# sunwookim028/bwa-mem-gpu

Measured on AMD Instinct MI355X. Metric: reads/s aligned (150 bp PE vs hg38-scale 3100 Mbp synthetic genome), file to file (bwahip_stream_run), higher is better.
Workload: dtype u64

## Files before the change

### bwa-mem-gpu_amd/bwahip.py

```python
import ctypes as C
import os
import subprocess
import numpy as np

_HERE = os.path.dirname(os.path.abspath(__file__))
LIB_PATH = os.environ.get("BWAHIP_LIB") or os.path.join(_HERE, "libbwahip.so")
TOOLS = os.path.join(_HERE, "tools")


class Opt(C.Structure):
    _fields_ = [("max_mem_intv", C.c_uint64), ("a", C.c_int), ("b", C.c_int), ("o_del", C.c_int), ("e_del", C.c_int),
                ("o_ins", C.c_int), ("e_ins", C.c_int), ("pen_unpaired", C.c_int), ("pen_clip5", C.c_int),
                ("pen_clip3", C.c_int), ("w", C.c_int), ("zdrop", C.c_int), ("T", C.c_int), ("flag", C.c_int),
                ("min_seed_len", C.c_int), ("min_chain_weight", C.c_int), ("max_chain_extend", C.c_int),
                ("split_factor", C.c_float), ("split_width", C.c_int), ("max_occ", C.c_int), ("max_chain_gap", C.c_int),
                ("n_threads", C.c_int), ("chunk_size", C.c_int), ("mask_level", C.c_float), ("drop_ratio", C.c_float),
                ("XA_drop_ratio", C.c_float), ("mask_level_redun", C.c_float), ("mapQ_coef_len", C.c_float),
                ("mapQ_coef_fac", C.c_int), ("max_ins", C.c_int), ("max_matesw", C.c_int), ("max_XA_hits", C.c_int),
                ("max_XA_hits_alt", C.c_int), ("mat", C.c_int8 * 25)]


class Seq(C.Structure):
    _fields_ = [("l_seq", C.c_int), ("id", C.c_int), ("name", C.c_char_p), ("comment", C.c_char_p),
                ("seq", C.POINTER(C.c_char)), ("qual", C.c_char_p), ("sam", C.POINTER(C.c_char)),
# ... 1169 lines not shown
        return dup[:len(desc)]

    def kat_radix_sort(self, keys, key_bits=64):
        keys = np.ascontiguousarray(keys, dtype=np.uint64)
        idx = np.empty(len(keys), dtype=np.uint32)
        tile = C.c_int()
        _check(lib().bwahip_kat_radix_sort(self._h, len(keys), keys.ctypes.data, key_bits, idx.ctypes.data, C.byref(tile)), "bwahip_kat_radix_sort")
        return idx, tile.value

    def batch_run(self, opt=None):
        opt = opt or default_opt()
        nk = lib().bwahip_n_kernels()
        ms = (C.c_float * nk)()
        _check(lib().bwahip_batch_run(self._h, C.byref(opt), ms, nk), "bwahip_batch_run")
        return {lib().bwahip_kernel_name(i).decode(): float(ms[i]) for i in range(nk)}

    @staticmethod
    def stage_names():
        return ["k_smem(passes 1-2)+k_smem_heavy+k_smem3(pass 3)+k_intv_sort", "k_seeds", "k_chain(+k_chain_big,k_chain_flt)", "k_seed_sw (only with -W / reads > 700 bp)",
                "k_extend_spec+k_extend(+k_extend_big, dedup/patch)", "pe_rescue = PE: k_pestat + k_pe_prepare + k_pe_copy (insert sizes, lists; the rescue kernels k_matesw_sw / k_matesw start on the second stream)",
                "k_mark (mark primary) + PE: k_pair (pairing) beside the rescue kernels, then both for the rescued pairs",
                "k_cigar (mem_reg2aln: mapQ, CIGAR by ksw_global2 backtrack, NM/MD)", "k_sam size + scan + write (SAM text)"]

    @staticmethod
    def output_description(paired):
        return "SAM text of the batch in HBM (== seqs[i].sam of mem_process_seqs, " + ("paired-end: mate rescue, pairing, paired records)" if paired else "single-end)")

    def counters(self):
        buf = (C.c_uint64 * 32)()
        _check(lib().bwahip_batch_counters(self._h, buf, 32), "bwahip_batch_counters")
        names = ["extend", "blocks", "sa", "lf", "intv", "seeds", "cells", "max_extends", "chain_build_max", "chain_sort_max", "chain_flt_max",
                 "chain_write_max", "max_seeds", "max_chains", "ext_max", "ext_dedup_max", "heavy_blocks", "heavy_intv", "heavy_reads",
                 "dp_rows_1col", "dp_rows_ncol", "dedup_sort1_max", "dedup_loop_max", "dedup_sort2_max",
                 "pass3_blocks", "pass3_intv", "pass3_jumped", "ext_calls", "ext_diag", "smem_lookups", "smem_fallbacks", "_31"]
        return {k: int(buf[i]) for i, k in enumerate(names)}

    def kat_introsort(self, k64, score, qb, mode):
        k64 = np.ascontiguousarray(k64, dtype=np.int64); score = np.ascontiguousarray(score, dtype=np.int32); qb = np.ascontiguousarray(qb, dtype=np.int32)
        n = len(k64)
        a = np.empty(n, dtype=np.int32); b = np.empty(n, dtype=np.int32); st = np.zeros(2, dtype=np.int32)
        _check(lib().bwahip_kat_introsort(self._h, n, mode, k64.ctypes.data, score.ctypes.data, qb.ctypes.data, a.ctypes.data, b.ctypes.data, st.ctypes.data), "bwahip_kat_introsort")
        assert st[1] == 0
        return a, b, bool(st[0])

    def kat_mate_insert(self, list_off, list_words, step_off, step_hit, step_words, opt=None, mode=0, where=0):
        opt = opt or default_opt()
        list_off = np.ascontiguousarray(list_off, dtype=np.int64); step_off = np.ascontiguousarray(step_off, dtype=np.int64)
        list_words = np.ascontiguousarray(list_words, dtype=np.int64).reshape(-1, 19); step_words = np.ascontiguousarray(step_words, dtype=np.int64).reshape(-1, 19)
        step_hit = np.ascontiguousarray(step_hit, dtype=np.int32)
        n = len(list_off) - 1
        assert len(step_off) == n + 1 and len(list_words) >= list_off.max() and len(step_words) >= step_off.max() and len(step_hit) == len(step_words)
        out = np.zeros((max(0, int(list_off[-1] + step_off[-1])), 19), dtype=np.int64); out_n = np.zeros(n, dtype=np.int32); cnt = np.zeros((n, 3), dtype=np.int32)
        _check(lib().bwahip_kat_mate_insert(self._h, C.byref(opt), n, list_off.ctypes.data, list_words.ctypes.data, step_off.ctypes.data, step_hit.ctypes.data, step_words.ctypes.data,
                                            mode, where, out.ctypes.data, out_n.ctypes.data, cnt.ctypes.data), "bwahip_kat_mate_insert")
        return out, out_n, cnt

    def kat_occ4(self, k):
        k = np.ascontiguousarray(k, dtype=np.uint64)
        out = np.zeros((len(k), 4), dtype=np.uint64)
        _check(lib().bwahip_kat_occ4(self._h, len(k), k.ctypes.data, out.ctypes.data), "bwahip_kat_occ4")
        return out

    def kat_sa(self, k):
        k = np.ascontiguousarray(k, dtype=np.uint64)
        out = np.zeros(len(k), dtype=np.uint64)
        _check(lib().bwahip_kat_sa(self._h, len(k), k.ctypes.data, out.ctypes.data), "bwahip_kat_sa")
        return out
# ... 284 lines not shown
```

### bwa-mem-gpu_amd/csrc/bwahip_internal.h

```cpp
#pragma once
#include <hip/hip_runtime.h>
#include <stdint.h>
#include <stdio.h>
#include <stdlib.h>
#include <string.h>
#include <vector>
#include <string>
#include "../../include/bwahip.h"

#define HIP_TRY(expr) do { hipError_t e_ = (expr); if (e_ != hipSuccess) { \
	fprintf(stderr, "[bwahip] %s failed at %s:%d: %s\n", #expr, __FILE__, __LINE__, hipGetErrorString(e_)); \
	return BWAHIP_ENODEV; } } while (0)

struct DevAnn { int64_t offset; int32_t len; int32_t is_alt; };

struct DevIndex {
	const uint4 *bwt;
	const uint64_t *sa;
	const uint8_t *pac;
	const DevAnn *anns;
	uint64_t primary, L2[5], seq_len, n_sa;
	int64_t l_pac;
	int sa_intv, sa_shift, n_seqs;
	const uint4 *kmer; int kmer_k;
};
__host__ __device__ inline uint64_t kmer_off(int L) { return (0x5555555555555555ull & ((1ull << 2 * L) - 1)) - 1; }

struct DevOpt {
	int a, b, o_del, e_del, o_ins, e_ins, pen_clip5, pen_clip3, w, zdrop;
	int min_seed_len, split_width, max_occ, max_chain_gap, max_mem_intv, split_len;
	int min_chain_weight, max_chain_extend;
	float mask_level, drop_ratio, mask_level_redun;
	int8_t mat[25];
	int T, flag, pen_unpaired, max_ins, max_matesw, max_XA_hits, max_XA_hits_alt, mapQ_coef_fac;
	float XA_drop_ratio, mapQ_coef_len;
};

enum { CNT_EXTEND = 0, CNT_BLOCKS, CNT_SA, CNT_LF, CNT_INTV, CNT_SEEDS, CNT_CELLS, CNT_MAX_EXT ,
       CNT_HEAVY_BLOCKS = 16, CNT_HEAVY_INTV, CNT_HEAVY_READS, CNT_ROWS1 , CNT_ROWSN ,
       CNT_P3_BLOCKS = 24, CNT_P3_INTV, CNT_P3_JUMPED ,
       CNT_EXT_CALLS , CNT_EXT_DIAG ,
       CNT_SMEM_LOOKUPS , CNT_SMEM_FALLBACKS , CNT_N = 32 };
constexpr int CNT_SLOTS = 256;
#define BWAHIP_MISC_BYTES ((size_t)CNT_SLOTS * CNT_N * 8 + 64)
#ifdef __HIPCC__
__device__ __forceinline__ unsigned long long *cnt_row(unsigned long long *base)
{
	return base + (size_t)((blockIdx.x * (blockDim.x >> 6) + (threadIdx.x >> 6)) & (CNT_SLOTS - 1)) * CNT_N;
}
#endif

struct __attribute__((aligned(32))) DevIntv { uint64_t x0, x1, x2, info; };

struct __attribute__((aligned(16))) DevSeed { int64_t rbeg; int32_t qbeg, len; int32_t score, rid; };

struct DevChain {
	int64_t pos;
	int32_t seed_off, n;
	int32_t rid, w, kept, first, is_alt;
	float frac_rep;
};

struct DevReg {
	int64_t rb, re;
	float frac_rep;
	int32_t qb, qe, rid, score, truesc, sub, csub, sub_n, w, seedcov, seedlen0, n_comp, is_alt;
	int32_t pad;
};

#include <thread>
#include <vector>
template <class F> static inline void par_for_chunks(int64_t n, int nt, F f)
{
	if (nt <= 1 || n < 4096) { f((int64_t)0, n); return; }
	std::vector<std::thread> th;
// ... 119 lines not shown
	int64_t pad2;
};
static_assert(sizeof(DevAln) == 80 && sizeof(DevReg) == 80, "record sizes");
enum { NEED_REC = 1 , NEED_XA = 2 , NEED_H = 4  };
struct DevPes { int low, high, failed, pad; double avg, std; };
struct PeRead;

struct FinLaunch {
	DevIndex ix; DevOpt opt;
	int n_reads; const uint8_t *seq; const int64_t *off;
	int64_t n_processed;
	const double *logtab;
	const DevReg *regs; const int64_t *reg_base; const int *reg_n;
	FinReg *fregs, *fregs2; int *freg_n, *n_pri; int *scr;
	const uint8_t *resc_flag; const int *resc_pairs; int subset;
	int read_lo;
	uint8_t *need; int *xa_owner;
	int *task_n, *rec_n;
	const int64_t *task_base;
	int2 *tasks;
	int *fast_list, *dp_list, *list_n;
	int *aln_of_reg;
	DevAln *alns;
	uint8_t *pool; unsigned long long *pool_head; unsigned long long pool_cap;
	int *redo_list, *redo_n; uint8_t *big_z;
	unsigned *zslab;
	const uint8_t *qual; const int64_t *qual_off;
	const uint8_t *names; const int64_t *name_off; const uint8_t *comments; const int64_t *comment_off;
	const uint8_t *ctg_names; const int *ctg_name_off; const uint8_t *ctg_anno; const int *ctg_anno_off;
	const uint8_t *rg_id; int rg_len;
	int *sam_len; const int64_t *sam_off; uint8_t *sam;
	const DevAln **rec_list, **xa_list;
	const PeRead *pe_read; DevPes pes[4];
	int *err;
};
int launch_mark_primary(const FinLaunch &a, bool plan, int n_listed, hipStream_t st);
int launch_kat_mapq(const FinLaunch &a, int64_t n_slots, int *out2, hipStream_t st);
int launch_task_fill(const FinLaunch &a, hipStream_t st);
int launch_cigar(const FinLaunch &a, int n_fast, int n_dp, int max_len, hipStream_t st, hipStream_t st2, hipEvent_t fork, hipEvent_t join);
int launch_cigar_big(const FinLaunch &a, int grid, hipStream_t st);
size_t cigar_big_slab_bytes();
size_t cigar_zslab_bytes(int max_len, int n_dp);
int launch_sam(const FinLaunch &a, bool write, hipStream_t st, int read_lo = 0, int read_hi = -1);

struct PeRead {
	int mode;
	int h_reg;
	int alt_reg;
	int mapq;
	int extra_flag;
	int pad[3];
};
struct SwRes { int state , score, te, qe, score2, te2, tb, qb; };
struct PairLaunch {
	DevIndex ix; DevOpt opt;
	int n_reads; const uint8_t *seq; const int64_t *off;
	int64_t n_processed;
	const double *logtab;
	const DevReg *regs; const int64_t *reg_base; const int *reg_n;
	unsigned *hist;
	DevPes pes[4];
	const double *pair_tab; int tab_off[4];
	int *nb;
	int *pe_cap; const int64_t *pe_base;
	DevReg *pe_regs; int *pe_n;
	DevReg *pe_tmp; void *pe_keys; int *pe_idx;
	int *resc_list; int *resc_n;
	const int64_t *sw_base; int *sw_cnt; SwRes *sw_res; int *sw_tasks; int2 *sw_info; int *sw_n;
	int *sw_n8; int sw_cap;
	uint8_t *slab; size_t slab_stride;
	int incr_insert;
	unsigned int *queue;
	unsigned long long *counters;
	unsigned long long *paths;
	int *pair_dbg;
// ... 59 lines not shown
```

### bwa-mem-gpu_amd/csrc/ctx_internal.h

```cpp
#pragma once
#include "bwahip_internal.h"
#include "own.h"
#include "upload_once.h"
#include <atomic>
#include <memory>
#include <string>
#include <utility>

inline std::atomic<long> g_bwahip_reallocs{0};
inline std::atomic<int64_t> g_bwahip_live[6];

struct DevMem {
	static constexpr size_t slack = 256;
	static constexpr const char *what = "hipMalloc";
	static void *alloc(size_t bytes)
	{
		void *p = nullptr;
		if (hipMalloc(&p, bytes ? bytes : 1) != hipSuccess) { (void)hipGetLastError(); return nullptr; }
		++g_bwahip_live[0]; g_bwahip_live[1] += (int64_t)bytes;
		return p;
	}
	static void free(void *p, size_t bytes) { (void)hipFree(p); --g_bwahip_live[0]; g_bwahip_live[1] -= (int64_t)bytes; }
	static void count_sync() { ++g_bwahip_reallocs; }
};
// ... 34 lines not shown
	Stream() = default;
	Stream(Stream &&o) noexcept : s(o.s) { o.s = nullptr; }
	Stream &operator=(Stream &&o) noexcept { if (this != &o) { reset(); s = o.s; o.s = nullptr; } return *this; }
	~Stream() { reset(); }
	int make(unsigned flags = hipStreamNonBlocking)
	{
		reset();
		if (hipStreamCreateWithFlags(&s, flags) != hipSuccess) { (void)hipGetLastError(); s = nullptr; return BWAHIP_ENODEV; }
		++g_bwahip_live[5];
		return 0;
	}
	void reset() { if (s) { (void)hipStreamDestroy(s); --g_bwahip_live[5]; s = nullptr; } }
	operator hipStream_t() const { return s; }
};

struct Knobs {
	int intv_cap = 96;
	int smem_lanes = 1;
	int sa_intv = 1;
	int kmer_k = 14;
	int smem_skip = -1;
	int heavy_mult = -1;
	int chain_mid_max = 1536, chain_big_max = 3200, chain_glb_grid = 2048;
	int chain_big_min = 512;
	int rank_sort_min = 2;
	int spec_min_chains = 16;
	int ext_lds_window = 1 << 30;
	int ext_early_stop = 1;
	int ext_diag = 1;
	int sorted_piece_blocks = 1024;
	int gpu_final = 1;
	int gpu_pair = 1;
	int incr_insert = 1;
	int verbose = 0;
	int e2e_log = 0;
	const char *dump_ext = nullptr;
	void from_env()
	{
		auto geti = [](const char *k, int &v) { if (const char *e = getenv(k)) v = atoi(e); };
		geti("BWAHIP_INTV_CAP", intv_cap); geti("BWAHIP_SMEM_LANES", smem_lanes); geti("BWAHIP_HEAVY_MULT", heavy_mult); geti("BWAHIP_SMEM_SKIP", smem_skip); geti("BWAHIP_SA_INTV", sa_intv); geti("BWAHIP_KMER_K", kmer_k);
		geti("BWAHIP_CHAIN_BIG_MIN", chain_big_min); geti("BWAHIP_CHAIN_MID_MAX", chain_mid_max); geti("BWAHIP_CHAIN_BIG_MAX", chain_big_max); geti("BWAHIP_CHAIN_GLB_GRID", chain_glb_grid); geti("BWAHIP_RANK_SORT_MIN", rank_sort_min); geti("BWAHIP_SPEC_MIN_CHAINS", spec_min_chains); geti("BWAHIP_EXT_LDS_WINDOW", ext_lds_window); geti("BWAHIP_EXT_EARLY_STOP", ext_early_stop); geti("BWAHIP_EXT_DIAG", ext_diag); geti("BWAHIP_GPU_FINAL", gpu_final); geti("BWAHIP_GPU_PAIR", gpu_pair);
		verbose = getenv("BWAHIP_VERBOSE") != nullptr;
		e2e_log = getenv("BWAHIP_E2E_LOG") != nullptr;
		dump_ext = getenv("BWAHIP_DUMP_EXT");
		if (intv_cap < 2) intv_cap = 2;
		ext_early_stop = ext_early_stop != 0; ext_diag = ext_diag != 0;
		geti("BWAHIP_INCR_INSERT", incr_insert); incr_insert = incr_insert != 0;
		geti("BWAHIP_SORTED_PIECE_BLOCKS", sorted_piece_blocks);
		if (sorted_piece_blocks < 1 || sorted_piece_blocks > 4096) sorted_piece_blocks = 1024;
	}
};

struct BatchText {
	std::vector<int64_t> off, qoff, noff, coff;
	int64_t qtot = 0;
	bool any_comment = false;
	size_t sz_codes = 0, sz_qual = 0, sz_names = 0, sz_comm = 0;
};

struct BamSort {
	DevBuf raw, rec_cnt, rec_base, keys[2], idx[2], off, len, len_sorted, hist, hist_base, bits;
	DevBuf tmpl;
	float ms[3] = { 0, 0, 0 };
	int n_passes = 0;
};

struct Bgzf {
	DevBuf slots, mlen, moff, md, cnt;
};

enum class OutForm { Sam, Bam, BamSorted, Bgzf, BamSortedDup };
inline bool is_bam(OutForm f) { return f != OutForm::Sam; }
inline bool is_sorted(OutForm f) { return f == OutForm::BamSorted || f == OutForm::BamSortedDup; }

struct BatchIn {
	DevBuf d_seq, d_off, d_qual, d_qual_off, d_names, d_name_off, d_comments, d_comment_off;
	HostBuf h_stage;
	Event ev;
	int n = 0, max_len = 0; int64_t total_bases = 0; bool any_comment = false;
	const uint8_t *comments() const { return any_comment ? d_comments.as<uint8_t>() : nullptr; }
// ... 205 lines not shown
```

### bwa-mem-gpu_amd/csrc/final_rt.hip

```cpp
#include "ctx_internal.h"
#include <atomic>
#include <thread>
#include <math.h>
#include <algorithm>
#include <chrono>

#include <dlfcn.h>
typedef int (*host_final_fn)(bwahip_ctx*, const bwahip_opt_t*, int64_t, int, bwahip_seq_t*, const bwahip_pestat_t*);
static host_final_fn load_host_final()
{
	static host_final_fn fn = nullptr;
	static bool tried = false;
	if (tried) return fn;
	tried = true;
	Dl_info di;
	std::string path = "libbwahip_hostfinal.so";
	if (dladdr((const void*)&bwahip_version, &di) && di.dli_fname) {
		const std::string self = di.dli_fname;
		const size_t sl = self.rfind('/');
		if (sl != std::string::npos) path = self.substr(0, sl + 1) + path;
	}
	void *h = dlopen(path.c_str(), RTLD_NOW | RTLD_LOCAL);
	if (h) fn = (host_final_fn)dlsym(h, "bwahip_process_seqs_host");
	if (!fn) fprintf(stderr, "[bwahip] gpu_final / gpu_pair = 0 need the test library %s (%s)\n", path.c_str(), h ? "symbol missing" : dlerror());
// ... 132 lines not shown
	HIP_TRY(hipMemcpyAsync(&n_sw_tasks, pl.sw_n, 4, hipMemcpyDeviceToHost, c->stream));
	HIP_TRY(hipStreamSynchronize(c->stream));
	n_resc_out = n_resc;
	c->last_pe_counters[3] = (unsigned long long)n_resc;
	c->last_sw_tasks = (unsigned long long)n_sw_tasks + (unsigned long long)n_sw_tasks8;
	c->last_sw_ahead[0] = (unsigned long long)n_sw_tasks; c->last_sw_ahead[1] = (unsigned long long)n_sw_tasks8;
	if (n_resc > 0 || n_sw_tasks > 0 || n_sw_tasks8 > 0) {
		HIP_TRY(hipEventRecord(c->ev_fork, c->stream));
		HIP_TRY(hipStreamWaitEvent(c->stream2, c->ev_fork, 0));
		if ((rc = launch_matesw_sw(pl, n_sw_tasks, n_sw_tasks8, c->in->max_len, c->stream2))) return rc;
		if (n_resc > 0) {
			if ((rc = c->d_resc_ord.ensure(((size_t)3 * n_resc + 8) * 4)) || (rc = launch_resc_order(pl, n_resc, c->d_resc_ord.as<int>(), c->stream2))) return rc;
			const int grid = std::min(n_resc, 2048);
			pl.slab_stride = (matesw_slab_bytes(widest + c->in->max_len) + 255) & ~(size_t)255;
			if ((rc = c->d_ms_slab.ensure(pl.slab_stride * (size_t)grid))) return rc;
			pl.slab = c->d_ms_slab.as<uint8_t>();
			HIP_TRY(hipMemsetAsync(pl.queue, 0, 16, c->stream2));
			if ((rc = launch_matesw(pl, grid, c->stream2))) return rc;
		}
		HIP_TRY(hipEventRecord(c->ev_join, c->stream2));
	}
	return 0;
}

static int mark_prepare(bwahip_ctx *c, const bwahip_opt_t *opt, int n, int64_t n_processed, bool pe_lists, FinLaunch &f)
{
	int rc;
	const size_t R = (size_t)(c->total_regs ? c->total_regs : 1);
	if ((rc = c->d_fregs.ensure(R * sizeof(FinReg))) || (rc = c->d_fregs2.ensure(R * sizeof(FinReg))) || (rc = c->d_fscr.ensure(R * 16)) || (rc = c->d_need.ensure(R)) ||
	    (rc = c->d_xa_owner.ensure(R * 4)) || (rc = c->d_freg_n.ensure((size_t)n * 4)) || (rc = c->d_npri.ensure((size_t)n * 4)) || (rc = c->d_task_n.ensure((size_t)n * 4)) ||
	    (rc = c->d_rec_n.ensure((size_t)n * 4))) return rc;
	memset(&f, 0, sizeof f);
	f.ix = c->ix; f.opt = make_dev_opt(opt); f.n_reads = n;
	f.n_processed = n_processed; f.logtab = c->d_logtab.as<double>();
	f.regs = c->d_regs.as<DevReg>(); f.reg_base = c->d_reg_base.as<int64_t>(); f.reg_n = c->d_reg_n.as<int>();
	if (pe_lists) { f.regs = c->d_pe_regs.as<DevReg>(); f.reg_base = c->d_pe_base.as<int64_t>(); f.reg_n = c->d_pe_n.as<int>(); }
	f.fregs = c->d_fregs.as<FinReg>(); f.fregs2 = c->d_fregs2.as<FinReg>(); f.freg_n = c->d_freg_n.as<int>(); f.n_pri = c->d_npri.as<int>(); f.scr = c->d_fscr.as<int>();
	f.need = c->d_need.as<uint8_t>(); f.xa_owner = c->d_xa_owner.as<int>(); f.task_n = c->d_task_n.as<int>(); f.rec_n = c->d_rec_n.as<int>();
	return 0;
}

static int pair_wire(bwahip_ctx *c, const FinLaunch &f, int n, bool dbg, PairLaunch &pl)
{
	int rc;
	if ((rc = c->d_pe_read.ensure((size_t)n * sizeof(PeRead)))) return rc;
	pl.fregs = f.fregs; pl.fregs_w = f.fregs; pl.fregs_tmp = f.fregs2; pl.freg_n = f.freg_n; pl.n_pri = f.n_pri; pl.need = f.need; pl.xa_owner = f.xa_owner;
	pl.task_n = f.task_n; pl.rec_n = f.rec_n; pl.scr = f.scr; pl.pe_read = c->d_pe_read.as<PeRead>();
	if (dbg) {
		if ((rc = c->d_pair_dbg.ensure((size_t)(n / 2) * 12))) return rc;
		HIP_TRY(hipMemsetAsync(c->d_pair_dbg.p, 0, (size_t)(n / 2) * 12, c->stream));
		pl.pair_dbg = c->d_pair_dbg.as<int>();
	}
	return 0;
}

int run_final(bwahip_ctx *c, const bwahip_opt_t *opt, int64_t n_processed, const bwahip_pestat_t *pes0, bool timed, OutForm form, bool host_sam_off, bool pe_stage_stop)
{
	auto launch_out = [&](const FinLaunch &fl, bool write, int lo, int hi) {
		const bool pe_ = (opt->flag & BWAHIP_F_PE) != 0;
		return is_bam(form) ? (pe_ ? launch_bam_pe(fl, write, c->stream, lo, hi) : launch_bam(fl, write, c->stream, lo, hi)) : (pe_ ? launch_sam_pe(fl, write, c->stream, lo, hi) : launch_sam(fl, write, c->stream, lo, hi));
	};
	const int n = c->in->n;
	const bool pe = (opt->flag & BWAHIP_F_PE) != 0;
	BatchOut &o = *c->out;
	o.total = 0; o.n_rec = 0; o.n_blocks = 0; o.n_stored = 0; o.n_tmpl = 0; o.form = form; c->total_tasks = 0;
	const bool sorted = is_sorted(form);
	const bool bgzf = form == OutForm::Bgzf;
	if (n == 0) return 0;
	if (pe && (n & 1)) return BWAHIP_EINVAL;
	int rc;
	HIP_TRY(hipMemsetAsync(c->d_fmisc.p, 0, 256, c->stream));
	if (timed) HIP_TRY(hipEventRecord(c->ev[20], c->stream));
	PairLaunch pl;
	const DevOpt dopt_pe = make_dev_opt(opt);
	int n_resc = 0;
	if (pe && (rc = run_pe_rescue(c, opt, dopt_pe, n_processed, pes0, pl, n_resc))) return rc;
	FinLaunch f;
	if ((rc = mark_prepare(c, opt, n, n_processed, pe, f))) return rc;
	const size_t R = (size_t)(c->total_regs ? c->total_regs : 1);
	if ((rc = c->d_aln_of_reg.ensure(R * 4)) || (rc = c->d_rec_list.ensure(R * 8)) || (rc = c->d_xa_list.ensure(R * 8)) ||
	    (rc = c->d_task_base.ensure((size_t)(n + 1) * 8)) || (rc = c->d_sam_len.ensure((size_t)n * 4)) || (rc = o.d_sam_off.ensure((size_t)(n + 1) * 8))) return rc;
	{
		std::string rg = c->rg_id;
		rg.resize(rg.size() + 64, 0);
		if ((rc = dev_upload(c->d_rg, rg.data(), rg.size(), c->stream))) return rc;
	}
	f.seq = c->in->d_seq.as<uint8_t>(); f.off = c->in->d_off.as<int64_t>();
	f.task_base = c->d_task_base.as<int64_t>(); f.aln_of_reg = c->d_aln_of_reg.as<int>();
	f.rec_list = c->d_rec_list.as<const DevAln*>(); f.xa_list = c->d_xa_list.as<const DevAln*>();
	unsigned long long *pool_head = c->d_fmisc.as<unsigned long long>();
	f.pool_head = pool_head; f.redo_n = (int*)(pool_head + 1); f.err = (int*)(pool_head + 2);
	f.qual = c->in->d_qual.as<uint8_t>(); f.qual_off = c->in->d_qual_off.as<int64_t>(); f.names = c->in->d_names.as<uint8_t>(); f.name_off = c->in->d_name_off.as<int64_t>();
	f.comments = c->in->comments(); f.comment_off = c->in->d_comment_off.as<int64_t>();
	f.ctg_names = c->d_ctg_names.as<uint8_t>(); f.ctg_name_off = c->d_ctg_name_off.as<int>(); f.ctg_anno = c->d_ctg_anno.as<uint8_t>(); f.ctg_anno_off = c->d_ctg_anno_off.as<int>();
	f.rg_id = c->d_rg.as<uint8_t>(); f.rg_len = (int)c->rg_id.size();
	f.sam_len = c->d_sam_len.as<int>(); f.sam_off = o.d_sam_off.as<int64_t>();
	if (timed) HIP_TRY(hipEventRecord(c->ev[15], c->stream));
	if (pe) { f.resc_flag = pl.resc_flag; f.resc_pairs = pl.resc_list; f.subset = 1; }
	if ((rc = launch_mark_primary(f, !pe, 0, c->stream))) return rc;
	if (pe) {
		if ((rc = pair_wire(c, f, n, pe_stage_stop, pl))) return rc;
		pl.subset = 1;
		if ((rc = launch_pair(pl, 0, c->stream))) return rc;
		HIP_TRY(hipStreamWaitEvent(c->stream, c->ev_join, 0));
		if (n_resc > 0) {
			f.subset = 2; pl.subset = 2;
			if ((rc = launch_mark_primary(f, false, n_resc, c->stream))) return rc;
			if ((rc = launch_pair(pl, n_resc, c->stream))) return rc;
		}
		f.subset = 0; pl.subset = 0;
		static_assert(bwahip_ctx::PE_CNT_PATHS == 19 - 5, "PairLaunch::paths starts at d_fmisc[19], the counters at [5]");
		HIP_TRY(hipMemcpyAsync(c->last_pe_counters, pl.counters, bwahip_ctx::PE_CNT_N * 8, hipMemcpyDeviceToHost, c->stream));
		f.pe_read = pl.pe_read;
		memcpy(f.pes, pl.pes, sizeof f.pes);
	}
	if (pe_stage_stop) {
		if (!pe) return BWAHIP_EINVAL;
		HIP_TRY(hipStreamSynchronize(c->stream));
		int err = 0;
		HIP_TRY(hipMemcpy(&err, c->d_fmisc.as<unsigned long long>() + 2, 4, hipMemcpyDeviceToHost));
		if (err) { fprintf(stderr, "[bwahip] paired-end kernels reported code %d\n", err); return BWAHIP_EINTERNAL; }
		return 0;
	}
	if ((rc = launch_scan(c->d_task_n.as<int>(), c->d_task_base.as<int64_t>(), n, c->d_scan, c->stream))) return rc;
	if (timed) HIP_TRY(hipEventRecord(c->ev[16], c->stream));
	int64_t T = 0;
	HIP_TRY(hipMemcpyAsync(&T, c->d_task_base.as<int64_t>() + n, 8, hipMemcpyDeviceToHost, c->stream));
	HIP_TRY(hipStreamSynchronize(c->stream));
	c->total_tasks = T;
	const size_t Tn = (size_t)(T ? T : 1);
	if ((rc = c->d_tasks.ensure(Tn * 8)) || (rc = c->d_alns.ensure(Tn * sizeof(DevAln))) || (rc = c->d_fredo.ensure((Tn + 4) * 4)) || (rc = c->d_task_lists.ensure(2 * Tn * 4))) return rc;
	f.tasks = c->d_tasks.as<int2>(); f.alns = c->d_alns.as<DevAln>(); f.redo_list = c->d_fredo.as<int>();
	f.fast_list = c->d_task_lists.as<int>(); f.dp_list = f.fast_list + Tn; f.list_n = (int*)(pool_head + 15);
	if ((rc = launch_task_fill(f, c->stream))) return rc;
	int n_list[2] = { 0, 0 };
	HIP_TRY(hipMemcpyAsync(n_list, f.list_n, 8, hipMemcpyDeviceToHost, c->stream));
	HIP_TRY(hipStreamSynchronize(c->stream));
	size_t want_pool = std::max(c->pool_cap, Tn * 64 + Tn * 32 + (size_t)(16 << 20));
	for (int attempt = 0;; ++attempt) {
		if ((rc = c->d_pool.ensure(want_pool))) return rc;
		c->pool_cap = want_pool;
		f.pool = c->d_pool.as<uint8_t>(); f.pool_cap = want_pool;
		HIP_TRY(hipMemsetAsync(c->d_fmisc.p, 0, 120, c->stream));
		{ const unsigned long long head0 = (unsigned long long)Tn * 64; HIP_TRY(hipMemcpyAsync(c->d_fmisc.p, &head0, 8, hipMemcpyHostToDevice, c->stream)); }
		if (n_list[1] > 0) { if ((rc = c->d_zslab.ensure(cigar_zslab_bytes(c->in->max_len, n_list[1])))) return rc; f.zslab = c->d_zslab.as<unsigned>(); }
		if ((rc = launch_cigar(f, n_list[0], n_list[1], c->in->max_len, c->stream, c->stream2, c->ev_fork, c->ev_join))) return rc;
		int h[6] = { 0 };
		HIP_TRY(hipMemcpyAsync(h, c->d_fmisc.p, 24, hipMemcpyDeviceToHost, c->stream));
		HIP_TRY(hipStreamSynchronize(c->stream));
		int n_redo = h[2], err = h[4];
		if (err == 5 && attempt < 6) { want_pool *= 4; continue; }
		if (!err && n_redo > 0) {
			const int grid = std::min(n_redo, 256);
			if ((rc = c->d_bigz.ensure((size_t)grid * cigar_big_slab_bytes()))) return rc;
			f.big_z = c->d_bigz.as<uint8_t>();
			if ((rc = launch_cigar_big(f, grid, c->stream))) return rc;
			HIP_TRY(hipMemcpyAsync(h, c->d_fmisc.p, 24, hipMemcpyDeviceToHost, c->stream));
			HIP_TRY(hipStreamSynchronize(c->stream));
			err = h[4];
			if (err == 5 && attempt < 6) { want_pool *= 4; continue; }
		}
		if (err) {
			fprintf(stderr, "[bwahip] alignment kernel reported code %d (read %d of the batch)%s\n", err, h[5], err == 6 ? ": a region's reference span / band exceeds the compiled limits" : "");
			return err == 6 ? BWAHIP_ECAPACITY : BWAHIP_EINTERNAL;
		}
		break;
	}
	if (timed) HIP_TRY(hipEventRecord(c->ev[17], c->stream));
	if ((rc = launch_out(f, false, 0, -1))) return rc;
	if ((rc = launch_scan(c->d_sam_len.as<int>(), o.d_sam_off.as<int64_t>(), n, c->d_scan, c->stream))) return rc;
	if (timed) HIP_TRY(hipEventRecord(c->ev[18], c->stream));
	int64_t total = 0;
	HIP_TRY(hipMemcpyAsync(&total, o.d_sam_off.as<int64_t>() + n, 8, hipMemcpyDeviceToHost, c->stream));
	HIP_TRY(hipStreamSynchronize(c->stream));
	o.total = total; if (bgzf) o.n_blocks = bgzf_blocks(total);
	if ((rc = o.d_sam.ensure((size_t)total + (bgzf ? (size_t)bgzf_blocks(total) * 31 : 0) + 64))) return rc;
	f.sam = o.d_sam.as<uint8_t>();
	if (sorted || bgzf) { if ((rc = c->bs.raw.ensure((size_t)total + 64))) return rc; f.sam = c->bs.raw.as<uint8_t>(); }
// ... 899 lines not shown
```

### bwa-mem-gpu_amd/csrc/k_final.hip

```cpp
#include "bwahip_internal.h"
#include "wave_dev.h"
#include "final_dev.h"

namespace {
using namespace wv;
using namespace fin;

__device__ __forceinline__ uint64_t hash_64(uint64_t key)
{
	key += ~(key << 32); key ^= (key >> 22); key += ~(key << 13); key ^= (key >> 8);
	key += (key << 3); key ^= (key >> 15); key += ~(key << 27); key ^= (key >> 31);
	return key;
}

struct SortKey { int score, is_alt; uint64_t hash; };
template <int MODE> __device__ __forceinline__ bool key_lt(const SortKey &a, const SortKey &b)
{
	if (MODE == 0) return a.score > b.score || (a.score == b.score && (a.is_alt < b.is_alt || (a.is_alt == b.is_alt && a.hash < b.hash)));
	return a.is_alt < b.is_alt || (a.is_alt == b.is_alt && (a.score > b.score || (a.score == b.score && a.hash < b.hash)));
}

__device__ void mark_core(const DevOpt &opt, int n, FinReg *f, int *z, int l)
{
	int tmp = opt.a + opt.b;
// ... 677 lines not shown
}

constexpr int CG_TCAP_SMALL = 768;
__host__ __device__ constexpr size_t cigar_zslab_words(int tcap) { return (size_t)(tcap + 72) * 16; }
template <bool FAST, int CPLMAX>
__global__ __launch_bounds__(64, FAST ? 7 : CPLMAX <= 3 ? 6 : 5) void k_cigar(FinLaunch a, int n_list)
{
	constexpr bool SMALL = FAST || CPLMAX <= 3;
	constexpr int TCAP = SMALL ? CG_TCAP_SMALL : CG_MAXT, MC = FAST ? 8 : SMALL ? 160 : CG_MAXC, MMD = SMALL ? 512 : CG_MAXMD;
	__shared__ uint8_t s_q[CG_MAXQ + 8];
	__shared__ uint8_t s_t[TCAP + 8];
	__shared__ uint8_t s_z[16];
	__shared__ uint32_t s_cig[MC];
	__shared__ uint8_t s_md[MMD];
	__shared__ int8_t s_mat[32];
	const int l = lane();
	if (l < 25) s_mat[l] = a.opt.mat[l];
	unsigned *zg = FAST ? nullptr : a.zslab + (size_t)blockIdx.x * cigar_zslab_words(TCAP);
	for (int it = (int)blockIdx.x; it < n_list; it += FAST ? n_list : (int)gridDim.x) {
		const long long t = FAST ? a.fast_list[it] : a.dp_list[it];
		const int2 tk = a.tasks[t];
		const int r = tk.x;
		const int l_query = (int)(a.off[r + 1] - a.off[r]);
		const uint8_t *query = a.seq + a.off[r];
		__syncthreads();
		for (int i = l; i < l_query; i += 64) { const uint8_t c = query[i]; s_q[i] = c < 5 ? c : 4; }
		__syncthreads();
		const FinReg ar = a.fregs[a.reg_base[r] + tk.y];
		const CigarLds m = { s_q, s_t, s_z, s_cig, s_md, s_mat, MC, MMD, zg };
		if (!reg2aln<false, FAST, CPLMAX>(a, ar, r, t, m, TCAP, 0, a.alns + t) && l == 0) a.redo_list[atomicAdd(a.redo_n, 1)] = (int)t;
	}
}

__global__ __launch_bounds__(64) void k_cigar_big(FinLaunch a)
{
	__shared__ uint8_t s_q[CG_MAXQ + 8];
	__shared__ uint32_t s_cig[CG_MAXC];
	__shared__ uint8_t s_md[CG_MAXMD];
	__shared__ int8_t s_mat[32];
	const int l = lane();
	uint8_t *slab = a.big_z + (size_t)blockIdx.x * (CG_BIG_Z + CG_BIG_T + 64);
	const int n_redo = *a.redo_n;
	for (int it = (int)blockIdx.x; it < n_redo; it += (int)gridDim.x) {
		const long long t = a.redo_list[it];
		const int2 tk = a.tasks[t];
		const int r = tk.x;
		const int l_query = (int)(a.off[r + 1] - a.off[r]);
		const uint8_t *query = a.seq + a.off[r];
		__syncthreads();
		for (int i = l; i < l_query; i += 64) { const uint8_t c = query[i]; s_q[i] = c < 5 ? c : 4; }
		if (l < 25) s_mat[l] = a.opt.mat[l];
		__syncthreads();
		const FinReg ar = a.fregs[a.reg_base[r] + tk.y];
		const CigarLds m = { s_q, slab + CG_BIG_Z, slab, s_cig, s_md, s_mat, CG_MAXC, CG_MAXMD };
		if (!reg2aln<true>(a, ar, r, t, m, CG_BIG_T, CG_BIG_Z, a.alns + t) && l == 0) { atomicExch(a.err, 6); atomicExch(a.err + 1, r); }
	}
}

template <int FORM>
__global__ __launch_bounds__(64) void k_kat_global(KatDp a, uint8_t *big_z, unsigned *zslab, int *out2, uint32_t *cig_out)
{
	__shared__ uint8_t s_q[CG_MAXQ + 8];
	__shared__ uint8_t s_t[CG_MAXT + 8];
	__shared__ uint8_t s_z[16];
	__shared__ uint32_t s_cig[CG_MAXC];
	__shared__ uint8_t s_md[16];
// ... 41 lines not shown
	if (grid <= 0) return 0;
	if (plan) hipLaunchKernelGGL(k_mark<true>, dim3(grid), dim3(64), 0, st, a);
	else hipLaunchKernelGGL(k_mark<false>, dim3(grid), dim3(64), 0, st, a);
	return hipGetLastError() == hipSuccess ? 0 : BWAHIP_ENODEV;
}

int launch_kat_mapq(const FinLaunch &a, int64_t n_slots, int *out2, hipStream_t st)
{
	if (n_slots <= 0) return 0;
	hipLaunchKernelGGL(k_kat_mapq, dim3((unsigned)((n_slots + 255) / 256)), dim3(256), 0, st, a, n_slots, out2);
	return hipGetLastError() == hipSuccess ? 0 : BWAHIP_ENODEV;
}

int launch_task_fill(const FinLaunch &a, hipStream_t st)
{
	if (a.n_reads <= 0) return 0;
	hipLaunchKernelGGL(k_task_fill, dim3((a.n_reads + 255) / 256), dim3(256), 0, st, a);
	return hipGetLastError() == hipSuccess ? 0 : BWAHIP_ENODEV;
}

size_t cigar_big_slab_bytes() { return CG_BIG_Z + CG_BIG_T + 64; }

size_t kat_global_zslab_bytes() { return cigar_zslab_words(CG_MAXT) * 4; }
int kat_global_t_cap(int form) { return form == 1 ? CG_BIG_T : CG_MAXT; }
int launch_kat_global(const KatDp &a, int form, int grid, uint8_t *big_z, unsigned *zslab, int *out2, uint32_t *cig_out, hipStream_t st)
{
	static_assert(CG_MAXC == BWAHIP_KAT_MAX_CIGAR, "the known-answer entry hands out CG_MAXC words per item");
	if (a.n <= 0) return 0;
	if (form == 1) hipLaunchKernelGGL(k_kat_global<1>, dim3(grid), dim3(64), 0, st, a, big_z, zslab, out2, cig_out);
	else hipLaunchKernelGGL(k_kat_global<0>, dim3(grid), dim3(64), 0, st, a, big_z, zslab, out2, cig_out);
	return hipGetLastError() == hipSuccess ? 0 : BWAHIP_ENODEV;
}

int cigar_dp_grid(int n_dp) { return n_dp < 256 * 28 ? n_dp : 256 * 28; }
size_t cigar_zslab_bytes(int max_len, int n_dp)
{
	return (size_t)cigar_dp_grid(n_dp) * cigar_zslab_words(max_len < 64 * 3 ? CG_TCAP_SMALL : CG_MAXT) * 4;
}
int launch_cigar(const FinLaunch &a, int n_fast, int n_dp, int max_len, hipStream_t st, hipStream_t st2, hipEvent_t fork, hipEvent_t join)
{
	const bool both = n_fast > 0 && n_dp > 0;
	if (both && (hipEventRecord(fork, st) != hipSuccess || hipStreamWaitEvent(st2, fork, 0) != hipSuccess)) return BWAHIP_ENODEV;
	if (n_dp > 0) {
		const unsigned grid = (unsigned)cigar_dp_grid(n_dp);
		if (max_len < 64 * 3) hipLaunchKernelGGL((k_cigar<false, 3>), dim3(grid), dim3(64), 0, st, a, n_dp);
		else if (max_len < 64 * 5) hipLaunchKernelGGL((k_cigar<false, 5>), dim3(grid), dim3(64), 0, st, a, n_dp);
		else hipLaunchKernelGGL((k_cigar<false, 11>), dim3(grid), dim3(64), 0, st, a, n_dp);
	}
	if (n_fast > 0) hipLaunchKernelGGL((k_cigar<true, 1>), dim3((unsigned)n_fast), dim3(64), 0, both ? st2 : st, a, n_fast);
	if (both && (hipEventRecord(join, st2) != hipSuccess || hipStreamWaitEvent(st, join, 0) != hipSuccess)) return BWAHIP_ENODEV;
	return hipGetLastError() == hipSuccess ? 0 : BWAHIP_ENODEV;
}

int launch_cigar_big(const FinLaunch &a, int grid, hipStream_t st)
{
	hipLaunchKernelGGL(k_cigar_big, dim3(grid), dim3(64), 0, st, a);
	return hipGetLastError() == hipSuccess ? 0 : BWAHIP_ENODEV;
}
```

### bwa-mem-gpu_amd/csrc/runtime.hip

```cpp
#include "ctx_internal.h"
#include <math.h>
#include <algorithm>
#include <atomic>

namespace {
constexpr int SCAN_T = 256, SCAN_PER = 16, SCAN_TILE = SCAN_T * SCAN_PER;

__device__ __forceinline__ long long block_excl_scan(long long v, long long *sh, long long *total)
{
	const int t = threadIdx.x;
	sh[t] = v;
	__syncthreads();
	for (int d = 1; d < SCAN_T; d <<= 1) {
		long long o = t >= d ? sh[t - d] : 0;
		__syncthreads();
		sh[t] += o;
		__syncthreads();
	}
	const long long incl = sh[t];
	*total = sh[SCAN_T - 1];
	__syncthreads();
	return incl - v;
}

// ... 314 lines not shown
{
	if (!out) return BWAHIP_EINVAL;
	for (int k = 0; k < 6; ++k) out[k] = g_bwahip_live[k].load();
	return 0;
}

int bwahip_ctx_set_rg_id(bwahip_ctx *c, const char *id) { if (!c) return BWAHIP_EINVAL; c->rg_id = id ? id : ""; return 0; }
const char *bwahip_ctx_rg_id(const bwahip_ctx *c) { return c ? c->rg_id.c_str() : ""; }
const bwahip_bns_t *bwahip_bns(const bwahip_ctx *c) { return c ? &c->host.bns : nullptr; }
const bwahip_bwt_t *bwahip_bwt(const bwahip_ctx *c) { return c ? &c->host.bwt : nullptr; }
const uint8_t *bwahip_pac(const bwahip_ctx *c) { return c ? c->host.pac : nullptr; }

int bwahip_ctx_tune(bwahip_ctx *c, const char *key, int value)
{
	if (!c || !key) return BWAHIP_EINVAL;
	Knobs &k = c->knobs;
	if (!strcmp(key, "intv_cap")) { k.intv_cap = value < 2 ? 2 : value; c->intv_cap = k.intv_cap; }
	else if (!strcmp(key, "smem_lanes")) { if (value != 1 && value != 2 && value != 4 && value != 8) return BWAHIP_EINVAL; k.smem_lanes = value; }
	else if (!strcmp(key, "heavy_mult")) k.heavy_mult = value;
	else if (!strcmp(key, "smem_skip")) { if (value < -1 || value == 1) return BWAHIP_EINVAL; k.smem_skip = value; }
	else if (!strcmp(key, "chain_big_min")) k.chain_big_min = value;
	else if (!strcmp(key, "chain_mid_max")) k.chain_mid_max = value;
	else if (!strcmp(key, "chain_big_max")) k.chain_big_max = value;
	else if (!strcmp(key, "chain_glb_grid")) { if (value < 1 || value > 65536) return BWAHIP_EINVAL; k.chain_glb_grid = value; }
	else if (!strcmp(key, "rank_sort_min")) k.rank_sort_min = value;
	else if (!strcmp(key, "spec_min_chains")) k.spec_min_chains = value;
	else if (!strcmp(key, "ext_lds_window")) k.ext_lds_window = value < 1 ? 1 : value;
	else if (!strcmp(key, "ext_early_stop")) { if (value != 0 && value != 1) return BWAHIP_EINVAL; k.ext_early_stop = value; }
	else if (!strcmp(key, "ext_diag")) { if (value != 0 && value != 1) return BWAHIP_EINVAL; k.ext_diag = value; }
	else if (!strcmp(key, "sorted_piece_blocks")) { if (value < 1 || value > 4096) return BWAHIP_EINVAL; k.sorted_piece_blocks = value; }
	else if (!strcmp(key, "gpu_final")) k.gpu_final = value;
	else if (!strcmp(key, "gpu_pair")) k.gpu_pair = value;
	else if (!strcmp(key, "incr_insert")) { if (value != 0 && value != 1) return BWAHIP_EINVAL; k.incr_insert = value; }
	else if (!strcmp(key, "verbose")) k.verbose = value;
	else return BWAHIP_EINVAL;
	return 0;
}

int bwahip_kat_ksw_align(bwahip_ctx *c, int n, const int *params, const int8_t *mat25, const uint8_t *q, const int64_t *qoff,
                         const uint8_t *t, const int64_t *toff, int *out7)
{
	if (!c || n < 0 || (n && (!params || !q || !qoff || !t || !toff || !out7))) return BWAHIP_EINVAL;
	if (n == 0) return 0;
	HIP_TRY(hipSetDevice(c->device));
	bwahip_opt_t o; bwahip_opt_init(&o);
	if (mat25) memcpy(o.mat, mat25, 25);
	DevOpt dopt = make_dev_opt(&o);
	std::vector<int> items[2];
	size_t stride = 0;
	for (int i = 0; i < n; ++i) {
		const int qlen = params[8*i], tlen = params[8*i+1];
		if (qlen < 0 || tlen < 0 || qlen > (1 << 20) || tlen > (1 << 20)) return BWAHIP_EINVAL;
		items[(params[8*i+2] & 0x10000) ? 1 : 0].push_back(i);
		const size_t cells = (size_t)(qlen + 15) / 16 * 16;
		stride = std::max(stride, 5 * cells + 16 + 8 * cells + 2 * (size_t)tlen + 16);
	}
	stride = (stride + 15) & ~(size_t)15;
	DevBuf dp, dq, dqo, dt, dto, dout, dit, dw; int rc;
	if ((rc = upload(dp, params, (size_t)n * 32, c->stream)) || (rc = upload(dq, q, (size_t)qoff[n], c->stream)) || (rc = upload(dqo, qoff, (size_t)(n + 1) * 8, c->stream)) ||
	    (rc = upload(dt, t, (size_t)toff[n], c->stream)) || (rc = upload(dto, toff, (size_t)(n + 1) * 8, c->stream)) || (rc = dout.ensure((size_t)n * 28)) ||
	    (rc = dw.ensure(stride * (size_t)n))) return rc;
	for (int m = 0; m < 2 && !rc; ++m) {
		if (items[m].empty()) continue;
		if ((rc = upload(dit, items[m].data(), items[m].size() * 4, c->stream))) break;
		rc = launch_kat_align(dopt, (int)items[m].size(), m, dit.as<int>(), dp.as<int>(), dq.as<uint8_t>(), dqo.as<int64_t>(), dt.as<uint8_t>(), dto.as<int64_t>(),
		                      dw.as<uint8_t>(), stride, dout.as<int>(), c->stream);
// ... 1026 lines not shown
```

Measured before the change: 14.66 million.

## Process fast-path CIGAR tasks four per wavefront and size DP grid to occupancy

Adds k_cigar_group, which handles ungapped (fast-list) CIGAR/MD tasks with 16-lane subgroups so one 64-lane block covers four alignments. Mismatches are found with ballots and the MD string is built in LDS. This replaces the one-block-per-task k_cigar<true,1> launch and is meant to cut idle lanes and launch overhead for short reads. For short reads the persistent DP cigar grid is also capped at CUs times max resident blocks, which shrinks the zslab. Long MD strings or oversized tasks fall back to the redo list, and a new counter tracks how many tasks took the grouped path.

```diff
diff --git a/bwa-mem-gpu_amd/bwahip.py b/bwa-mem-gpu_amd/bwahip.py
--- a/bwa-mem-gpu_amd/bwahip.py
+++ b/bwa-mem-gpu_amd/bwahip.py
@@ -1225,7 +1225,7 @@
         names = ["extend", "blocks", "sa", "lf", "intv", "seeds", "cells", "max_extends", "chain_build_max", "chain_sort_max", "chain_flt_max",
                  "chain_write_max", "max_seeds", "max_chains", "ext_max", "ext_dedup_max", "heavy_blocks", "heavy_intv", "heavy_reads",
                  "dp_rows_1col", "dp_rows_ncol", "dedup_sort1_max", "dedup_loop_max", "dedup_sort2_max",
-                 "pass3_blocks", "pass3_intv", "pass3_jumped", "ext_calls", "ext_diag", "smem_lookups", "smem_fallbacks", "_31"]
+                 "pass3_blocks", "pass3_intv", "pass3_jumped", "ext_calls", "ext_diag", "smem_lookups", "smem_fallbacks", "cigar_group_tasks"]
         return {k: int(buf[i]) for i, k in enumerate(names)}
 
     def kat_introsort(self, k64, score, qb, mode):
diff --git a/bwa-mem-gpu_amd/csrc/bwahip_internal.h b/bwa-mem-gpu_amd/csrc/bwahip_internal.h
--- a/bwa-mem-gpu_amd/csrc/bwahip_internal.h
+++ b/bwa-mem-gpu_amd/csrc/bwahip_internal.h
@@ -40,7 +40,9 @@
        CNT_HEAVY_BLOCKS = 16, CNT_HEAVY_INTV, CNT_HEAVY_READS, CNT_ROWS1 , CNT_ROWSN ,
        CNT_P3_BLOCKS = 24, CNT_P3_INTV, CNT_P3_JUMPED ,
        CNT_EXT_CALLS , CNT_EXT_DIAG ,
-       CNT_SMEM_LOOKUPS , CNT_SMEM_FALLBACKS , CNT_N = 32 };
+       CNT_SMEM_LOOKUPS , CNT_SMEM_FALLBACKS ,
+       CNT_CIGAR_GROUP , CNT_N = 32 };
+static_assert(CNT_CIGAR_GROUP == 31, "bwahip_batch_counters documents these indices");
 constexpr int CNT_SLOTS = 256;
 #define BWAHIP_MISC_BYTES ((size_t)CNT_SLOTS * CNT_N * 8 + 64)
 #ifdef __HIPCC__
@@ -226,6 +228,8 @@
 	int *sam_len; const int64_t *sam_off; uint8_t *sam;
 	const DevAln **rec_list, **xa_list;
 	const PeRead *pe_read; DevPes pes[4];
+	int final_lane;
+	unsigned long long *counters;
 	int *err;
 };
 int launch_mark_primary(const FinLaunch &a, bool plan, int n_listed, hipStream_t st);
@@ -234,7 +238,7 @@
 int launch_cigar(const FinLaunch &a, int n_fast, int n_dp, int max_len, hipStream_t st, hipStream_t st2, hipEvent_t fork, hipEvent_t join);
 int launch_cigar_big(const FinLaunch &a, int grid, hipStream_t st);
 size_t cigar_big_slab_bytes();
-size_t cigar_zslab_bytes(int max_len, int n_dp);
+size_t cigar_zslab_bytes(int max_len, int n_dp, int final_lane);
 int launch_sam(const FinLaunch &a, bool write, hipStream_t st, int read_lo = 0, int read_hi = -1);
 
 struct PeRead {
diff --git a/bwa-mem-gpu_amd/csrc/ctx_internal.h b/bwa-mem-gpu_amd/csrc/ctx_internal.h
--- a/bwa-mem-gpu_amd/csrc/ctx_internal.h
+++ b/bwa-mem-gpu_amd/csrc/ctx_internal.h
@@ -90,6 +90,7 @@
 	int gpu_final = 1;
 	int gpu_pair = 1;
 	int incr_insert = 1;
+	int final_lane = 1;
 	int verbose = 0;
 	int e2e_log = 0;
 	const char *dump_ext = nullptr;
@@ -104,6 +105,7 @@
 		if (intv_cap < 2) intv_cap = 2;
 		ext_early_stop = ext_early_stop != 0; ext_diag = ext_diag != 0;
 		geti("BWAHIP_INCR_INSERT", incr_insert); incr_insert = incr_insert != 0;
+		geti("BWAHIP_FINAL_LANE", final_lane); final_lane = final_lane != 0;
 		geti("BWAHIP_SORTED_PIECE_BLOCKS", sorted_piece_blocks);
 		if (sorted_piece_blocks < 1 || sorted_piece_blocks > 4096) sorted_piece_blocks = 1024;
 	}
diff --git a/bwa-mem-gpu_amd/csrc/final_rt.hip b/bwa-mem-gpu_amd/csrc/final_rt.hip
--- a/bwa-mem-gpu_amd/csrc/final_rt.hip
+++ b/bwa-mem-gpu_amd/csrc/final_rt.hip
@@ -188,7 +188,7 @@
 	    (rc = c->d_rec_n.ensure((size_t)n * 4))) return rc;
 	memset(&f, 0, sizeof f);
 	f.ix = c->ix; f.opt = make_dev_opt(opt); f.n_reads = n;
-	f.n_processed = n_processed; f.logtab = c->d_logtab.as<double>();
+	f.n_processed = n_processed; f.logtab = c->d_logtab.as<double>(); f.final_lane = c->knobs.final_lane;
 	f.regs = c->d_regs.as<DevReg>(); f.reg_base = c->d_reg_base.as<int64_t>(); f.reg_n = c->d_reg_n.as<int>();
 	if (pe_lists) { f.regs = c->d_pe_regs.as<DevReg>(); f.reg_base = c->d_pe_base.as<int64_t>(); f.reg_n = c->d_pe_n.as<int>(); }
 	f.fregs = c->d_fregs.as<FinReg>(); f.fregs2 = c->d_fregs2.as<FinReg>(); f.freg_n = c->d_freg_n.as<int>(); f.n_pri = c->d_npri.as<int>(); f.scr = c->d_fscr.as<int>();
@@ -245,7 +245,7 @@
 	f.task_base = c->d_task_base.as<int64_t>(); f.aln_of_reg = c->d_aln_of_reg.as<int>();
 	f.rec_list = c->d_rec_list.as<const DevAln*>(); f.xa_list = c->d_xa_list.as<const DevAln*>();
 	unsigned long long *pool_head = c->d_fmisc.as<unsigned long long>();
-	f.pool_head = pool_head; f.redo_n = (int*)(pool_head + 1); f.err = (int*)(pool_head + 2);
+	f.pool_head = pool_head; f.redo_n = (int*)(pool_head + 1); f.err = (int*)(pool_head + 2); f.counters = c->d_misc.as<unsigned long long>();
 	f.qual = c->in->d_qual.as<uint8_t>(); f.qual_off = c->in->d_qual_off.as<int64_t>(); f.names = c->in->d_names.as<uint8_t>(); f.name_off = c->in->d_name_off.as<int64_t>();
 	f.comments = c->in->comments(); f.comment_off = c->in->d_comment_off.as<int64_t>();
 	f.ctg_names = c->d_ctg_names.as<uint8_t>(); f.ctg_name_off = c->d_ctg_name_off.as<int>(); f.ctg_anno = c->d_ctg_anno.as<uint8_t>(); f.ctg_anno_off = c->d_ctg_anno_off.as<int>();
@@ -299,7 +299,7 @@
 		f.pool = c->d_pool.as<uint8_t>(); f.pool_cap = want_pool;
 		HIP_TRY(hipMemsetAsync(c->d_fmisc.p, 0, 120, c->stream));
 		{ const unsigned long long head0 = (unsigned long long)Tn * 64; HIP_TRY(hipMemcpyAsync(c->d_fmisc.p, &head0, 8, hipMemcpyHostToDevice, c->stream)); }
-		if (n_list[1] > 0) { if ((rc = c->d_zslab.ensure(cigar_zslab_bytes(c->in->max_len, n_list[1])))) return rc; f.zslab = c->d_zslab.as<unsigned>(); }
+		if (n_list[1] > 0) { if ((rc = c->d_zslab.ensure(cigar_zslab_bytes(c->in->max_len, n_list[1], f.final_lane)))) return rc; f.zslab = c->d_zslab.as<unsigned>(); }
 		if ((rc = launch_cigar(f, n_list[0], n_list[1], c->in->max_len, c->stream, c->stream2, c->ev_fork, c->ev_join))) return rc;
 		int h[6] = { 0 };
 		HIP_TRY(hipMemcpyAsync(h, c->d_fmisc.p, 24, hipMemcpyDeviceToHost, c->stream));
diff --git a/bwa-mem-gpu_amd/csrc/k_final.hip b/bwa-mem-gpu_amd/csrc/k_final.hip
--- a/bwa-mem-gpu_amd/csrc/k_final.hip
+++ b/bwa-mem-gpu_amd/csrc/k_final.hip
@@ -733,6 +733,109 @@
 	}
 }
 
+constexpr int CG_GROUP_MD = 512;
+__device__ __forceinline__ int put_dec(uint8_t *dst, unsigned v, bool store)
+{
+	int n = 1;
+	for (unsigned x = v; x >= 10; x /= 10) ++n;
+	if (store) for (int k = n - 1; k >= 0; --k) { dst[k] = (uint8_t)('0' + v % 10); v /= 10; }
+	return n;
+}
+__global__ __launch_bounds__(64, 7) void k_cigar_group(FinLaunch a, int n_list)
+{
+	__shared__ uint8_t s_md[4][CG_GROUP_MD];
+	const int l = lane(), g = l >> 4, gl = l & 15, gsh = g << 4;
+	const int it = (int)blockIdx.x * 4 + g;
+	if (l == 0 && a.counters) { const int left = n_list - (int)blockIdx.x * 4; atomicAdd(&cnt_row(a.counters)[CNT_CIGAR_GROUP], (unsigned long long)(left < 4 ? left : 4)); }
+	if (it >= n_list) return;
+	const long long t = a.fast_list[it];
+	const int2 tk = a.tasks[t];
+	const int r = tk.x;
+	const int64_t q0 = a.off[r];
+	const int l_query = (int)(a.off[r + 1] - q0);
+	const uint8_t *query = a.seq + q0;
+	const FinReg ar = a.fregs[a.reg_base[r] + tk.y];
+	const DevOpt &opt = a.opt;
+	const DevIndex &ix = a.ix;
+	const int64_t l_pac = ix.l_pac;
+	const int qb = ar.qb, qe = ar.qe, lq = qe - qb;
+	const int64_t rb = ar.rb, re = ar.re;
+	if (lq <= 0 || rb >= re || (rb < l_pac && re > l_pac)) { if (gl == 0) atomicExch(a.err, 30); return; }
+	if (qb < 0 || qe > l_query || (int64_t)lq != re - rb || lq > CG_TCAP_SMALL) { if (gl == 0) a.redo_list[atomicAdd(a.redo_n, 1)] = (int)t; return; }
+	const bool rev = rb >= l_pac;
+	int bad = 0;
+	DevAln al;
+	al.flag = ar.secondary >= 0 ? 0x100 : 0;
+	al.mapq = ar.secondary < 0 ? (uint32_t)approx_mapq_se(opt, a.logtab, ar, &bad) & 0xff : 0;
+	if (bad && gl == 0) atomicExch(a.err, 31);
+	uint8_t *md = s_md[g];
+	const unsigned int2base = rev ? ('T' | 'G' << 8 | 'C' << 16 | 'A' << 24) : ('A' | 'C' << 8 | 'G' << 16 | 'T' << 24);
+	int md_len = 0, n_mm = 0, u = 0;
+	bool md_ovf = false;
+	for (int base = 0; base < lq; base += 64) {
+		int qv[4], tv[4];
+#pragma unroll
+		for (int c = 0; c < 4; ++c) {
+			const int i = base + 16 * c + gl, ic = i < lq ? i : lq - 1;
+			qv[c] = query[rev ? qe - 1 - ic : qb + ic];
+			tv[c] = ref_base(ix, rev ? re - 1 - ic : rb + ic);
+		}
+		unsigned long long mm = 0;
+		unsigned tpack = 0;
+#pragma unroll
+		for (int c = 0; c < 4; ++c) {
+			const int i = base + 16 * c + gl;
+			const int qc = qv[c] < 5 ? qv[c] : 4;
+			mm |= (__ballot(i < lq && qc != tv[c]) >> gsh & 0xffffull) << (16 * c);
+			tpack |= (unsigned)tv[c] << (4 * c);
+		}
+		int prev = 0;
+		while (mm) {
+			const int p = __ffsll((long long)mm) - 1;
+			mm &= mm - 1;
+			u += p - prev;
+			if (md_len + 11 < CG_GROUP_MD) md_len += put_dec(md + md_len, (unsigned)u, gl == 0); else md_ovf = true;
+			const int tb = __shfl((int)tpack, p & 15, 16) >> ((p >> 4) << 2) & 3;
+			if (md_len + 1 < CG_GROUP_MD) { if (gl == 0) md[md_len] = (uint8_t)(int2base >> (tb << 3)); ++md_len; } else md_ovf = true;
+			++n_mm; u = 0; prev = p + 1;
+		}
+		const int chunk = lq - base < 64 ? lq - base : 64;
+		u += chunk - prev;
+	}
+	if (md_len + 11 < CG_GROUP_MD) md_len += put_dec(md + md_len, (unsigned)u, gl == 0); else md_ovf = true;
+	if (md_ovf) { if (gl == 0) a.redo_list[atomicAdd(a.redo_n, 1)] = (int)t; return; }
+	__threadfence_block();
+	al.NM = (uint32_t)n_mm & 0x3fffff;
+	const int is_rev = rev ? 1 : 0;
+	const int64_t pos = rev ? (l_pac << 1) - 1 - (re - 1) : rb;
+	int clip5 = 0, clip3 = 0;
+	if (qb != 0 || qe != l_query) { clip5 = is_rev ? l_query - qe : qb; clip3 = is_rev ? qb : l_query - qe; }
+	const int n_out = 1 + (clip5 ? 1 : 0) + (clip3 ? 1 : 0);
+	al.is_rev = (uint32_t)is_rev;
+	al.rid = dev_pos2rid(ix, pos);
+	al.pos = pos - ix.anns[al.rid].offset;
+	al.score = ar.score; al.sub = ar.sub > ar.csub ? ar.sub : ar.csub;
+	al.is_alt = (uint32_t)ar.is_alt; al.alt_sc = ar.alt_sc;
+	al.n_cigar = n_out; al.md_len = md_len; al.pad = 0; al.pad2 = 0;
+	const unsigned long long bytes = ((unsigned long long)n_out * 4 + (unsigned long long)md_len + 7) & ~7ull;
+	unsigned long long at = (unsigned long long)t * CG_SLOT;
+	if (bytes > CG_SLOT) {
+		if (gl == 0) at = atomicAdd(a.pool_head, bytes);
+		at = (unsigned long long)__shfl((long long)at, 0, 16);
+		if (at + bytes > a.pool_cap) { if (gl == 0) atomicExch(a.err, 5); return; }
+	}
+	uint32_t *dc = reinterpret_cast<uint32_t*>(a.pool + at);
+	if (gl == 0) {
+		if (clip5) dc[0] = (uint32_t)clip5 << 4 | 3;
+		dc[clip5 ? 1 : 0] = (uint32_t)lq << 4 | 0;
+		if (clip3) dc[n_out - 1] = (uint32_t)clip3 << 4 | 3;
+	}
+	uint8_t *dm = a.pool + at + (size_t)n_out * 4;
+	for (int i = gl; i < md_len; i += 16) dm[i] = md[i];
+	al.cigar_off = (int64_t)at; al.md_off = (int64_t)(at + (unsigned long long)n_out * 4);
+	if (gl == 0) a.alns[t] = al;
+}
+
 __global__ __launch_bounds__(64) void k_cigar_big(FinLaunch a)
 {
 	__shared__ uint8_t s_q[CG_MAXQ + 8];
@@ -840,22 +943,35 @@
 	return hipGetLastError() == hipSuccess ? 0 : BWAHIP_ENODEV;
 }
 
-int cigar_dp_grid(int n_dp) { return n_dp < 256 * 28 ? n_dp : 256 * 28; }
-size_t cigar_zslab_bytes(int max_len, int n_dp)
-{
-	return (size_t)cigar_dp_grid(n_dp) * cigar_zslab_words(max_len < 64 * 3 ? CG_TCAP_SMALL : CG_MAXT) * 4;
+int cigar_dp_grid(int n_dp, int max_len, int final_lane)
+{
+	int g = 256 * 28;
+	if (final_lane && max_len < 64 * 3) {
+		int dev = 0, cus = 0, per_cu = 0;
+		hipError_t e = hipGetDevice(&dev);
+		if (e == hipSuccess) e = hipDeviceGetAttribute(&cus, hipDeviceAttributeMultiprocessorCount, dev);
+		if (e == hipSuccess) e = hipOccupancyMaxActiveBlocksPerMultiprocessor(&per_cu, k_cigar<false, 3>, 64, 0);
+		if (e != hipSuccess) (void)hipGetLastError();
+		else if (cus > 0 && per_cu > 0 && (long long)cus * per_cu < g) g = cus * per_cu;
+	}
+	return n_dp < g ? n_dp : g;
+}
+size_t cigar_zslab_bytes(int max_len, int n_dp, int final_lane)
+{
+	return (size_t)cigar_dp_grid(n_dp, max_len, final_lane) * cigar_zslab_words(max_len < 64 * 3 ? CG_TCAP_SMALL : CG_MAXT) * 4;
 }
 int launch_cigar(const FinLaunch &a, int n_fast, int n_dp, int max_len, hipStream_t st, hipStream_t st2, hipEvent_t fork, hipEvent_t join)
 {
 	const bool both = n_fast > 0 && n_dp > 0;
 	if (both && (hipEventRecord(fork, st) != hipSuccess || hipStreamWaitEvent(st2, fork, 0) != hipSuccess)) return BWAHIP_ENODEV;
 	if (n_dp > 0) {
-		const unsigned grid = (unsigned)cigar_dp_grid(n_dp);
+		const unsigned grid = (unsigned)cigar_dp_grid(n_dp, max_len, a.final_lane);
 		if (max_len < 64 * 3) hipLaunchKernelGGL((k_cigar<false, 3>), dim3(grid), dim3(64), 0, st, a, n_dp);
 		else if (max_len < 64 * 5) hipLaunchKernelGGL((k_cigar<false, 5>), dim3(grid), dim3(64), 0, st, a, n_dp);
 		else hipLaunchKernelGGL((k_cigar<false, 11>), dim3(grid), dim3(64), 0, st, a, n_dp);
 	}
-	if (n_fast > 0) hipLaunchKernelGGL((k_cigar<true, 1>), dim3((unsigned)n_fast), dim3(64), 0, both ? st2 : st, a, n_fast);
+	if (n_fast > 0 && a.final_lane) hipLaunchKernelGGL(k_cigar_group, dim3((unsigned)((n_fast + 3) / 4)), dim3(64), 0, both ? st2 : st, a, n_fast);
+	else if (n_fast > 0) hipLaunchKernelGGL((k_cigar<true, 1>), dim3((unsigned)n_fast), dim3(64), 0, both ? st2 : st, a, n_fast);
 	if (both && (hipEventRecord(join, st2) != hipSuccess || hipStreamWaitEvent(st, join, 0) != hipSuccess)) return BWAHIP_ENODEV;
 	return hipGetLastError() == hipSuccess ? 0 : BWAHIP_ENODEV;
 }
diff --git a/bwa-mem-gpu_amd/csrc/runtime.hip b/bwa-mem-gpu_amd/csrc/runtime.hip
--- a/bwa-mem-gpu_amd/csrc/runtime.hip
+++ b/bwa-mem-gpu_amd/csrc/runtime.hip
@@ -370,6 +370,7 @@
 	else if (!strcmp(key, "gpu_final")) k.gpu_final = value;
 	else if (!strcmp(key, "gpu_pair")) k.gpu_pair = value;
 	else if (!strcmp(key, "incr_insert")) { if (value != 0 && value != 1) return BWAHIP_EINVAL; k.incr_insert = value; }
+	else if (!strcmp(key, "final_lane")) { if (value != 0 && value != 1) return BWAHIP_EINVAL; k.final_lane = value; }
 	else if (!strcmp(key, "verbose")) k.verbose = value;
 	else return BWAHIP_EINVAL;
 	return 0;
```

Result: no change. 14.86 million, median of 6 (+1.4%).
